# bobochow/adapt-image-models

Measured on AMD Instinct MI355X. Metric: clips/sec (8-frame 224^2 ViT-B/16 AIM fwd+bwd), higher is better.
Workload: dtype bf16; 1 GPU; BASELINE configs[1]: ViT-B/16 + AIM adapters, 8 frames 224^2, 64 clips/GPU, K400-shaped synthetic clips (400 random labels), fwd+bwd+AdamW; global_batch=64, frames=8, parallelism=dp1

## Files before the change

adapt-image-models_amd/backbone.py:

```python
import logging
import os
from collections import OrderedDict
from typing import Dict, List, Optional

import torch
from torch import nn

from . import ops
from .registry import BACKBONES

BF16, F32 = torch.bfloat16, torch.float32
_LOG = logging.getLogger("aim_amd")


def get_root_logger():
    return _LOG


class Adapter(nn.Module):

    def __init__(self, D_features: int, mlp_ratio: float = 0.25, skip_connect: bool = True):
        super().__init__()
        self.skip_connect = skip_connect
        hidden = int(D_features * mlp_ratio)
# ... 494 lines not shown
        ctx = dict(top=True, mean1c=mean1.view(BT, N)[:, 0].contiguous(), rstd1c=rstd1.view(BT, N)[:, 0].contiguous())
    elif save:
        ctx = {}
    if save:
        ctx.update(x=x, mean1=mean1, rstd1=rstd1, qkv=qkv, probs=probs, ta=ta, t_pre=t_pre, t_h=t_h, lam=lam,
                   oml=oml, ao=ao, lse=lse, sin=sin, s_pre=s_pre, s_h=s_h, x1=x1, mean2=mean2, rstd2=rstd2, xn=xn,
                   hcat_pre=hcat_pre, a_s=a_s, dms1=dms1, dms2=dms2)
    return x2, ctx


def _mlp_adapter_forward(x1, fz: _Frozen, dms2, N, save: bool, small_tile: bool = False):
    dev = x1.device
    M, D = x1.shape
    r, H4 = fz.r, 4 * D
    xn = _empty((M, D), BF16, dev)
    mean2, rstd2 = _empty((M,), F32, dev), _empty((M,), F32, dev)
    ops.layernorm_fwd(x1, fz.g2, fz.b2, M, D, D, y_bf16=xn, mean=mean2, rstd=rstd2)
    frag = _AUX_FRAG and M >= 1024 and not small_tile
    if frag:
        hcat_pre = ops.frag_buffer(M, H4 + r, dev) if save else None
    else:
        hcat_pre = _empty((M, H4 + r), BF16, dev) if (save or M < 1024 or small_tile) else None
    hcat = _empty((M, H4 + r), BF16, dev)
    ops.gemm(xn, fz.Wcat1, ops.EPI_ACT, hcat, bias=fz.bcat1, out2=hcat_pre, act=ops.ACT_QGELU, n_split=H4,
             act2=ops.ACT_GELU, at=dms2, ntok=N, aux_grad=_AUX_GRAD, aux_frag=frag and hcat_pre is not None,
             small_tile=small_tile)
    x2 = _empty((M, D), F32, dev)
    ops.gemm(hcat, fz.Wcat2, ops.EPI_F32, x2, bias=fz.bpr, resid=x1, vec=fz.b2row, ldv=0, bt=dms2, ntok=N, small_tile=small_tile)
    a_s = hcat[:, H4:] if save else None
    return x2, xn, mean2, rstd2, hcat_pre, a_s


def _mlp_adapter_backward(dyb, x_in, mean2, rstd2, xn, hcat_pre, a_s, dms2, fz: _Frozen, gm, N, fsum=None,
                          small_tile: bool = False):
    dev = dyb.device
    M, D = dyb.shape
    r, H4 = fz.r, 4 * D
    big_later: list = []
    if _DETACH_BIG:
        big_later.append(lambda: ops.wgrad(dyb, a_s, gm["D_fc2.weight"], gm["D_fc2.bias"], at=dms2, ntok=N))
    else:
        ops.wgrad(dyb, a_s, gm["D_fc2.weight"], gm["D_fc2.bias"], at=dms2, ntok=N)
    dcat = _empty((M, H4 + r), BF16, dev)
    ops.gemm(dyb, fz.WcatT2, ops.EPI_DACT, dcat, aux=hcat_pre, act=ops.ACT_QGELU, n_split=H4, act2=ops.ACT_GELU,
             at=dms2, ntok=N, aux_grad=_AUX_GRAD, aux_frag=_AUX_FRAG and dyb.shape[0] >= 1024 and not small_tile,
             reserve_cus=_DP_RESERVE, small_tile=small_tile)
    if _DETACH_BIG:
        big_later.append(lambda: ops.wgrad(dcat[:, H4:], xn, gm["D_fc1.weight"], gm["D_fc1.bias"]))
    else:
        ops.wgrad(dcat[:, H4:], xn, gm["D_fc1.weight"], gm["D_fc1.bias"])
    dxn = _empty((M, D), BF16, dev)
    ops.gemm(dcat, fz.WcatT1, ops.EPI_BF16, dxn, reserve_cus=_DP_RESERVE, small_tile=small_tile)
    dxb = _empty((M, D), BF16, dev)
    if fsum is not None:
        ops.layernorm_bwd_fsum(dxn, x_in, fz.g2, mean2, rstd2, dyb, dxb, fsum[0], fsum[1], M // N, N, D)
    else:
        ops.layernorm_bwd(dxn, x_in, fz.g2, mean2, rstd2, M, D, lddy=D, ldx=D, lddx=D, dres=dyb, dx_bf16=dxb)
    return dxb, big_later


def _adapter_bwd_small(dout_bf, ad: _AdapterW, a_in, pre, h, grads, rows, r, D, ar: _Arena, need_dx_bf16: bool, later: list):
    later.append(lambda: ops.wgrad(dout_bf, h, grads["D_fc2.weight"], grads["D_fc2.bias"]))
    dpre = ar.take((rows, r), BF16)
    ops.gemm(dout_bf, ad.W2T, ops.EPI_DACT, dpre, aux=pre, act=ops.ACT_GELU, aux_grad=_AUX_GRAD)
    later.append(lambda: ops.wgrad(dpre, a_in, grads["D_fc1.weight"], grads["D_fc1.bias"]))
    din = ar.take((rows, D), BF16 if need_dx_bf16 else F32)
    ops.gemm(dpre, ad.W1T, ops.EPI_BF16 if need_dx_bf16 else ops.EPI_F32, din)
    return din


def _block_backward(dyb, c, fz: _Frozen, adp: Dict[str, _AdapterW], grads, B, T, N, H, keep: Optional[list] = None):
    dev = dyb.device
    D = dyb.shape[1]
    BT = B * T
    M = BT * N
    r, H4 = fz.r, 4 * D
    top = bool(c.get("top"))
    fsum_in_ln = _FSUM_IN_LN and not top
    fpart = _empty((BT, ops.LN_FSUM_GROUPS, D), F32, dev) if fsum_in_ln else None
    if top:
        dx1b, big_later = _mlp_adapter_backward(dyb, c["x1"], c["mean2"], c["rstd2"], c["xn"], c["hcat_pre"], c["a_s"],
                                                c["dms2"][:1], fz, grads["MLP_Adapter"], 1, small_tile=True)
    else:
        dx1b, big_later = _mlp_adapter_backward(dyb, c["x1"], c["mean2"], c["rstd2"], c["xn"], c["hcat_pre"], c["a_s"], c["dms2"],
                                                fz, grads["MLP_Adapter"], N, fsum=(c["dms1"], fpart) if fsum_in_ln else None)
    later: list = big_later
    ar = _Arena(dev, 48 * BT * D + (1 << 16))
    with _Fork(dev, "bwd") as fork:
        dsv = ar.take((BT, D), F32)
        if fsum_in_ln:
            ops.frame_sum(fpart, None, dsv, BT, ops.LN_FSUM_GROUPS, D)
        elif top:
            ops.frame_sum(dx1b, c["dms1"][:1], dsv, BT, 1, D)
        else:
            ops.frame_sum(dx1b, c["dms1"], dsv, BT, N, D)
        dsv_b = ar.take((BT, D), BF16)
        ops.cast_bf16(dsv, dsv_b)
        dsin = _adapter_bwd_small(dsv_b, adp["S_Adapter"], c["sin"], c["s_pre"], c["s_h"], grads["S_Adapter"], BT, r,
                                  D, ar, need_dx_bf16=False, later=later)
        dcrs = ar.take((BT, D), BF16)
        ops.scale_rows(dsin, c["lam"], y=dcrs)
        dvx = ar.take((BT, D), BF16)
        ops.gemm(dcrs, fz.WoT, ops.EPI_BF16, dvx)
        dxt = ar.take((BT, D), BF16)
        ops.gemm(dvx, fz.WqkvT[:, 2 * D:], ops.EPI_BF16, dxt)
        dta = _adapter_bwd_small(dxt, adp["T_Adapter"], c["ta"], c["t_pre"], c["t_h"], grads["T_Adapter"], BT, r, D,
                                 ar, need_dx_bf16=True, later=later)
        dot = ar.take((BT, D), BF16)
        ops.gemm(dta, fz.WoT, ops.EPI_BF16, dot)
        if _LATE_JOIN:
            dqkv_cls = ar.take((BT, 3 * D), BF16)
            ops.cls_attn_bwd(c["qkv"], c["probs"], dot, dqkv_cls, B, T, N, H, compact=True)
            dxl_cls = ar.take((BT, D), F32)
            ops.gemm(dqkv_cls, fz.WqkvT, ops.EPI_F32, dxl_cls)
    if keep is None:
        keep = []
        fork.run_detached(later, keep)
        _Fork.join_detached(dev)
    else:
        fork.run_detached(later, keep)
    dqkv = _empty((M, 3 * D), BF16, dev)
    if top:
        dao = _empty((BT, D), BF16, dev)
        ops.gemm(dx1b, fz.WoT, ops.EPI_BF16, dao, af=c["oml"], ntok=1, small_tile=True)
        ops.attn_bwd_cls(c["qkv"], c["ao"], dao, c["lse"], dqkv, BT, N, H)
    else:
        dao = _empty((M, D), BF16, dev)
        ops.gemm(dx1b, fz.WoT, ops.EPI_BF16, dao, af=c["oml"], ntok=N, reserve_cus=_DP_RESERVE)
        delta = _empty((BT, H, N), F32, dev)
        ops.attn_bwd(c["qkv"], c["ao"], dao, c["lse"], delta, dqkv, BT, N, H)
    del dao
    if not _LATE_JOIN:
        fork.join()
        ops.cls_attn_bwd(c["qkv"], c["probs"], dot, dqkv, B, T, N, H)
    dxl = _empty((M, D), BF16, dev)
    ops.gemm(dqkv, fz.WqkvT, ops.EPI_BF16, dxl, reserve_cus=_DP_RESERVE)
    del dqkv
    if _LATE_JOIN:
        fork.join()
        ops.add_rows(dxl, N * D, dxl_cls)
    dxb = _empty((M, D), BF16, dev)
    if top:
        ops.layernorm_bwd(dxl, c["x"], fz.g1, c["mean1"], c["rstd1"], M, D, lddy=D, ldx=D, lddx=D, dx_bf16=dxb)
        ops.layernorm_bwd(dxl, c["x"], fz.g1, c["mean1c"], c["rstd1c"], BT, D, lddy=N * D, ldx=N * D, lddx=N * D, dres=dx1b,
                          lddres=D, dx_bf16=dxb)
    else:
        ops.layernorm_bwd(dxl, c["x"], fz.g1, c["mean1"], c["rstd1"], M, D, lddy=D, ldx=D, lddx=D, dres=dx1b, dx_bf16=dxb)
# ... 397 lines not shown
```

adapt-image-models_amd/csrc/wgrad.hip:

```cpp
#include "aim_common.h"
#include <stdlib.h>
#include "aim_kernels_internal.h"

namespace {

constexpr int MSTEP = 32;
constexpr int NST = 4;
constexpr int IMG = MSTEP * 128;
constexpr int OPER_BYTES = 4 * IMG;
constexpr int STAGE_BYTES = 2 * OPER_BYTES;
constexpr int TILE = 256;

__global__ __launch_bounds__(512) void wgrad_kernel(const bf16_t* __restrict__ G, int ldg, const bf16_t* __restrict__ A,
                                                    int lda, float* __restrict__ dW, int lddw, float* __restrict__ partial,
                                                    int M, int Nw, int Kw, int chunk, float* __restrict__ db,
                                                    float* __restrict__ bias_partial, const float* __restrict__ at, int ntok) {
    extern __shared__ __attribute__((aligned(16))) char smem_raw[];
    AIM_LDS char* smem = (AIM_LDS char*)smem_raw;
    AIM_LDS float* sAt = (AIM_LDS float*)(smem + NST * STAGE_BYTES);
    const int tiles_k = (Kw + TILE - 1) / TILE;
    const int tiles = ((Nw + TILE - 1) / TILE) * tiles_k;
    const int cidx = blockIdx.x / tiles, tix = blockIdx.x - cidx * tiles;
    const int tn = tix / tiles_k, tk = tix - tn * tiles_k;
    const int n0 = tn * TILE, k0 = tk * TILE;
    const int mbeg = cidx * chunk;
    const int mend = min(M, mbeg + chunk);
    if (mbeg >= mend) return;

    const int tid = threadIdx.x, lane = tid & 63;
    const int wave = __builtin_amdgcn_readfirstlane(tid >> 6);
    const int wn = wave >> 2, wk = wave & 3;
    const int frow = lane & 15, fq = lane >> 4;

    const bf16_t* Gb = G + (long long)mbeg * ldg + n0;
    const bf16_t* Ab = A + (long long)mbeg * lda + k0;
    const int rows = mend - mbeg;
    aim_rsrc_words rG = make_rsrc_words(Gb, ((long long)(rows - 1) * ldg + min(TILE, Nw - n0)) * 2);
    aim_rsrc_words rA = make_rsrc_words(Ab, ((long long)(rows - 1) * lda + min(TILE, Kw - k0)) * 2);

    const int srow = lane >> 3, schunk = (lane & 7) ^ srow;
    unsigned vg0[2], va0[2];
    AIM_LDS char* pdst[2];
#pragma unroll
    for (int j = 0; j < 2; ++j) {
        const int piece = wave * 2 + j;
        const int img = piece >> 2, rg = piece & 3;
        const int r = rg * 8 + srow;
        const int col = img * 64 + schunk * 8;
        vg0[j] = n0 + col < Nw ? (unsigned)((r * ldg + col) * 2) : AIM_OOB;
        va0[j] = k0 + col < Kw ? (unsigned)((r * lda + col) * 2) : AIM_OOB;
        pdst[j] = smem + img * IMG + rg * 1024;
    }
    const unsigned gstep = (unsigned)(MSTEP * ldg * 2), astep = (unsigned)(MSTEP * lda * 2);
    auto stage = [&](int buf, int ms) {
#pragma unroll
        for (int j = 0; j < 2; ++j) {
            stage_piece_asm(rG, pdst[j] + buf * STAGE_BYTES, vg0[j] + (unsigned)ms * gstep);
            stage_piece_asm(rA, pdst[j] + buf * STAGE_BYTES + OPER_BYTES, va0[j] + (unsigned)ms * astep);
        }
// ... 106 lines not shown
            f32x4 v[8];
#pragma unroll
            for (int j = 0; j < 8; ++j) v[j] = *(const f32x4*)(partial + (long long)(c + j) * total + idx);
#pragma unroll
            for (int j = 0; j < 8; ++j) acc += v[j];
        }
        for (; c < nchunks; ++c) acc += *(const f32x4*)(partial + (long long)c * total + idx);
        const int n = (int)(idx / Kw), k = (int)(idx - (long long)n * Kw);
        f32x4* o = (f32x4*)(dW + (long long)n * lddw + k);
        *o = *o + acc;
    }
    if (bias_partial) {
        const int n = blockIdx.x * 4 + (threadIdx.x >> 6), lane = threadIdx.x & 63;
        if (n < Nw) {
            float a = 0.f;
            for (int c = lane; c < nchunks; c += 64) a += bias_partial[(long long)c * Nw + n];
            a = wave_sum(a);
            if (lane == 0) db[n] += a;
        }
    }
}

__global__ __launch_bounds__(256) void wgrad_finish1_kernel(const float* __restrict__ partial, float* __restrict__ dW,
                                                            int lddw, int nchunks, int Nw, int Kw) {
    const long long idx = (long long)blockIdx.x * 256 + threadIdx.x;
    const long long total = (long long)Nw * Kw;
    if (idx >= total) return;
    float acc = 0.f;
    for (int c = 0; c < nchunks; ++c) acc += partial[(long long)c * total + idx];
    const int n = (int)(idx / Kw), k = (int)(idx - (long long)n * Kw);
    dW[(long long)n * lddw + k] += acc;
}

}

static int wgrad_chunks(int M, int tiles, int* chunk_out) {
    static const int target = [] { const char* e = getenv("AIM_WGRAD_WGS"); const int v = e ? atoi(e) : 256; return v > 0 ? v : 256; }();
    int nchunks = (target + tiles - 1) / tiles;
    const int maxchunks = (M + MSTEP - 1) / MSTEP;
    if (nchunks > maxchunks) nchunks = maxchunks;
    int chunk = (M + nchunks - 1) / nchunks;
    chunk = ((chunk + MSTEP - 1) / MSTEP) * MSTEP;
    if (chunk_out) *chunk_out = chunk;
    return (M + chunk - 1) / chunk;
}

extern "C" int64_t aim_wgrad_workspace_bytes(int M, int Nw, int Kw) {
    const int tiles = ((Nw + TILE - 1) / TILE) * ((Kw + TILE - 1) / TILE);
    const int nchunks = wgrad_chunks(M, tiles, nullptr);
    return nchunks > 1 ? (int64_t)nchunks * Nw * (Kw + 1) * 4 : 0;
}

extern "C" int aim_wgrad_bias_bf16(const aim_bf16* G, int ldg, const aim_bf16* A, int lda, float* dW, int lddw, float* db,
                                   const float* at, int ntok, int M, int Nw, int Kw, float* workspace, int64_t workspace_bytes,
                                   void* stream) {
    AIM_CHECK_ARG(M > 0 && Nw > 0 && Kw > 0 && (Nw % 8) == 0 && (Kw % 8) == 0, "wgrad: Nw/Kw must be positive multiples of 8 (Nw=%d Kw=%d)", Nw, Kw);
    AIM_CHECK_ARG((ldg % 8) == 0 && (lda % 8) == 0 && (lddw % 4) == 0, "wgrad: ldg/lda must be multiples of 8, lddw of 4");
    AIM_CHECK_ARG(G && A && dW, "wgrad: null pointer");
    AIM_CHECK_ARG(!at || (db && ntok > 0 && ntok <= 4096), "wgrad: row factors need db and 0 < ntok <= 4096");
    const int tiles = ((Nw + TILE - 1) / TILE) * ((Kw + TILE - 1) / TILE);
    int chunk = 0;
    const int nchunks = wgrad_chunks(M, tiles, &chunk);
    const int lds_bytes = NST * STAGE_BYTES + (at ? ((ntok * 4 + 15) & ~15) : 0);
    static bool attr_set = false;
    if (!attr_set) {
        (void)hipFuncSetAttribute((const void*)wgrad_kernel, hipFuncAttributeMaxDynamicSharedMemorySize, 160 * 1024);
        attr_set = true;
    }
    AIM_CHECK_ARG((long long)chunk * (ldg > lda ? ldg : lda) * 2 < 0x7fffffffLL, "wgrad: chunk too large");
    float* slab = (workspace && nchunks > 1 && workspace_bytes >= (int64_t)nchunks * Nw * (Kw + 1) * 4) ? workspace : nullptr;
    static const bool fuse_bias = [] { const char* e = getenv("AIM_WGRAD_FUSE_BIAS"); return !e || atoi(e) != 0; }();
    static const bool finish_v = [] { const char* e = getenv("AIM_WGRAD_FINISH_V"); return !e || atoi(e) != 0; }();
    float* bias_slab = (slab && db && fuse_bias) ? slab + (long long)nchunks * Nw * Kw : nullptr;
    if (db && nchunks > 1 && !bias_slab) {
        const int rc = aim_colsum_bf16(G, ldg, nullptr, at, ntok, db, M, Nw, nullptr, 0, stream);
        if (rc) return rc;
        db = nullptr;
    }
    hipLaunchKernelGGL(wgrad_kernel, dim3(tiles * nchunks), dim3(512), lds_bytes, (hipStream_t)stream,
                       (const bf16_t*)G, ldg, (const bf16_t*)A, lda, dW, lddw, slab, M, Nw, Kw, chunk, db, bias_slab, at, ntok);
    AIM_CHECK_LAUNCH("aim_wgrad_bf16");
    if (slab) {
        const long long total = (long long)Nw * Kw;
        unsigned fgrid = (unsigned)((total / 4 + 255) / 256);
        if (bias_slab && (unsigned)((Nw + 3) / 4) > fgrid) fgrid = (unsigned)((Nw + 3) / 4);
        if (finish_v || bias_slab)
            hipLaunchKernelGGL(wgrad_finish_kernel, dim3(fgrid), dim3(256), 0, (hipStream_t)stream,
                               slab, dW, lddw, nchunks, Nw, Kw, bias_slab, db);
        else
            hipLaunchKernelGGL(wgrad_finish1_kernel, dim3((unsigned)((total + 255) / 256)), dim3(256), 0, (hipStream_t)stream,
                               slab, dW, lddw, nchunks, Nw, Kw);
        AIM_CHECK_LAUNCH("aim_wgrad_bf16(finish)");
    }
    return 0;
}

extern "C" int aim_wgrad_bf16(const aim_bf16* G, int ldg, const aim_bf16* A, int lda, float* dW, int lddw, float* db,
                              int M, int Nw, int Kw, float* workspace, int64_t workspace_bytes, void* stream) {
    return aim_wgrad_bias_bf16(G, ldg, A, lda, dW, lddw, db, nullptr, 0, M, Nw, Kw, workspace, workspace_bytes, stream);
}
```

adapt-image-models_amd/lib.py:

```python
import ctypes
import os
from ctypes import POINTER, Structure, c_char_p, c_float, c_int, c_int32, c_int64, c_void_p

_HERE = os.path.dirname(os.path.abspath(__file__))
_LIB = None


class LibraryNotBuilt(RuntimeError):
    pass


def library_path() -> str:
    return os.environ.get("AIM_HIP_LIB") or os.path.join(_HERE, "libaim_hip.so")


class GemmArgs(Structure):
    _fields_ = [
        ("A", c_void_p), ("W", c_void_p), ("lda", c_int32), ("ldw", c_int32),
        ("strideA", c_int64), ("strideW", c_int64),
        ("M", c_int32), ("N", c_int32), ("K", c_int32),
        ("bias", c_void_p), ("resid", c_void_p), ("ldr", c_int32),
        ("af", c_void_p), ("at", c_void_p), ("vec", c_void_p), ("bt", c_void_p),
        ("ldv", c_int32), ("ntok", c_int32),
        ("aux", c_void_p), ("ldaux", c_int32),
        ("out", c_void_p), ("ldo", c_int32), ("out2", c_void_p), ("ldo2", c_int32),
        ("scale", c_float), ("act", c_int32), ("rs_bias_only", c_int32), ("n_split", c_int32), ("act2", c_int32),
        ("xrow", c_void_p), ("ldx", c_int32),
        ("reserve_cus", c_int32), ("probe", c_void_p), ("probe_cap", c_int32),
        ("wscale", c_void_p), ("aux_grad", c_int32), ("aux_frag", c_int32), ("row0", c_int32),
        ("small_tile", c_int32),
    ]


P = c_void_p
I = c_int
L = c_int64
F = c_float

SIGNATURES = {
    "aim_version": [],
    "aim_last_error": [],
    "aim_gemm_bf16": [POINTER(GemmArgs), I, I, P],
    "aim_gemm_fp8": [POINTER(GemmArgs), I, P],
    "aim_gemm_expsum_tiles": [I, I],
    "aim_wgrad_bf16": [P, I, P, I, P, I, P, I, I, I, P, L, P],
    "aim_wgrad_workspace_bytes": [I, I, I],
    "aim_wgrad_bias_bf16": [P, I, P, I, P, I, P, P, I, I, I, I, P, L, P],
    "aim_layernorm_fwd": [P, L, P, P, P, P, L, P, P, I, I, F, P],
    "aim_layernorm_fwd_fp8": [P, L, P, P, P, L, I, I, F, P],
    "aim_layernorm_fwd_x16": [P, L, P, P, P, P, P, L, I, I, F, P],
    "aim_layernorm_bwd": [P, I, L, P, L, P, P, P, P, I, L, P, P, L, P, P, I, I, P],
    "aim_layernorm_bwd_fsum": [P, L, P, L, P, P, P, P, P, L, P, P, I, I, I, I, P],
    "aim_attn_fwd": [P, P, P, I, I, I, P],
    "aim_attn_fwd_fp8": [P, P, P, I, I, I, P],
    "aim_attn_bwd": [P, P, P, P, P, P, I, I, I, P],
    "aim_attn_fwd_cls": [P, P, P, I, I, I, P],
    "aim_attn_bwd_cls": [P, P, P, P, P, I, I, I, P],
    "aim_cls_attn_fwd": [P, P, P, I, I, I, I, P],
    "aim_cls_attn_bwd": [P, P, P, P, I, I, I, I, I, P],
    "aim_tattn_fwd": [P, P, P, I, I, I, I, P],
    "aim_tattn_bwd": [P, P, P, P, I, I, I, I, P],
    "aim_add_bf16": [P, L, P, L, P, L, I, I, P],
    "aim_acc_bf16": [P, P, L, I, I, P],
    "aim_lambda_partials": [P, P, P, I, P],
    "aim_qk_cross": [P, P, I, P, I, I, I, F, P],
    "aim_lambda": [P, P, I, P, P, I, P, P, I, I, I, F, P],
    "aim_qk_border": [P, P, I, P, P, I, I, I, I, I, F, P],
    "aim_patchify": [P, I, P, P, P, I, I, I, I, I, I, P],
    "aim_patchify_blend": [P, I, P, P, P, I, I, I, I, I, I, P, I, F, F, I, I, I, I, P],
    "aim_embed_ln": [P, P, P, P, P, P, P, P, P, I, I, I, I, F, P],
    "aim_embed_bwd": [P, I, P, P, P, P, P, P, P, P, I, I, I, I, P, L, P],
    "aim_embed_bwd_workspace_bytes": [I, I, I, I],
    "aim_frame_sum": [P, I, P, P, I, I, I, P],
    "aim_colsum_bf16": [P, I, P, P, I, P, I, I, P, L, P],
    "aim_cast_bf16": [P, P, I, I, I, I, P],
    "aim_scale_rows": [P, P, P, P, I, I, P],
    "aim_add_rows_bf16": [P, L, P, I, I, P],
    "aim_adamw_flat": [P, P, P, P, L, F, F, F, F, F, I, F, P],
    "aim_head_fwd": [P, P, P, P, P, P, I, I, I, I, P],
    "aim_head_bwd": [P, P, P, P, P, P, P, I, I, I, I, P],
    "aim_ce_topk": [P, P, P, P, P, I, I, I, P],
    "aim_ce_soft": [P, P, P, P, P, P, I, I, P],
    "aim_cast_multi": [P, I, P],
    "aim_gemm_f32": [POINTER(GemmArgs), I, I, P],
    "aim_attn_fwd_f32": [P, P, I, I, I, P],
    "aim_cls_attn_fwd_f32": [P, L, P, I, I, I, P],
    "aim_lambda_f32": [P, I, P, P, I, P, P, I, I, I, F, P],
    "aim_patchify_f32": [P, I, P, P, P, I, I, I, I, I, I, P],
    "aim_patchify_blend_f32": [P, I, P, P, P, I, I, I, I, I, I, P, I, F, F, I, I, I, I, P],
    "aim_embed_ln_f32": [P, P, P, P, P, P, P, P, P, P, I, I, I, I, F, P],
    "aim_attn_bwd_f32_workspace_bytes": [I, I, I],
    "aim_attn_bwd_f32": [P, P, P, I, I, I, P, L, P],
    "aim_cls_attn_bwd_f32": [P, L, P, P, I, I, I, P],
    "aim_tattn_fwd_f32": [P, P, I, I, I, I, P],
    "aim_tattn_bwd_f32": [P, P, P, I, I, I, I, P],
    "aim_wgrad_f32_workspace_bytes": [I, I, I],
    "aim_wgrad_f32": [P, I, P, I, P, I, I, I, P, P, I, P, L, P],
    "aim_embed_nopre_fwd": [P, P, P, P, P, I, I, I, I, P],
    "aim_embed_nopre_bwd_workspace_bytes": [I, I, I, I],
    "aim_embed_nopre_bwd": [P, I, P, P, P, P, P, I, I, I, I, P, L, P],
    "aim_layernorm_gb_bwd_workspace_bytes": [I, I],
    "aim_layernorm_gb_bwd": [P, I, L, P, L, P, P, P, P, I, I, P, L, P],
}

ABI_VERSION = 9


def load_library():
    global _LIB
    if _LIB is not None:
        return _LIB
    path = library_path()
    if not os.path.exists(path):
        raise LibraryNotBuilt(
            f"{path} not found: build it with `python -c 'import __graft_entry__ as g; g.build()'` "
            f"(or `make -C adapt-image-models_amd/csrc`). There is no CPU fallback.")
    lib = ctypes.CDLL(path)
    for name, argtypes in SIGNATURES.items():
        fn = getattr(lib, name)
        fn.argtypes = argtypes
        fn.restype = c_char_p if name == "aim_last_error" else (c_int64 if name.endswith("_bytes") else c_int)
    if lib.aim_version() != ABI_VERSION:
        raise LibraryNotBuilt(f"{path}: ABI version {lib.aim_version()} != {ABI_VERSION}; rebuild")
    _LIB = lib
    return lib


def check(rc: int, what: str = ""):
    if rc != 0:
        msg = load_library().aim_last_error()
        raise RuntimeError(f"libaim_hip {what} failed (rc={rc}): {msg.decode() if msg else '?'}")
```

adapt-image-models_amd/ops.py:

```python
from ctypes import byref
from typing import Optional

import torch

from .lib import GemmArgs, check, load_library

EPI_BF16, EPI_ACT, EPI_DACT, EPI_F32, EPI_EXPSUM, EPI_ACT8, EPI_RES16 = 0, 1, 2, 3, 4, 5, 6
FP8 = torch.float8_e4m3fn
ACT_QGELU, ACT_GELU = 0, 1

BF16 = torch.bfloat16
F32 = torch.float32


_RAW_STREAM = getattr(torch._C, "_cuda_getCurrentRawStream", None)
_RAW_DEVICE = getattr(torch._C, "_cuda_getDevice", None)


def _stream() -> int:
    if _RAW_STREAM is not None:
        return _RAW_STREAM(_RAW_DEVICE())
    return torch.cuda.current_stream().cuda_stream


class KernelTimer:

    def __init__(self, min_flops: float = 1e10):
        self.min_flops = min_flops
        self.enabled = False
        self.records = []

    def start(self):
        self.records, self.enabled = [], True

    def stop(self):
        self.enabled = False

    def summary(self):
# ... 152 lines not shown
    check(load_library().aim_layernorm_fwd_fp8(x.data_ptr(), ldx, gamma.data_ptr(), beta.data_ptr(), y8.data_ptr(),
                                               D if ldy is None else ldy, rows, D, eps, _stream()), "aim_layernorm_fwd_fp8")


def layernorm_fwd_x16(x, gamma, beta, rows, D, ldx, *, y_bf16=None, y_f32=None, y8=None, ldy=None, eps: float = 1e-5):
    _chk(x, BF16, "x"); _chk(gamma, F32, "gamma"); _chk(beta, F32, "beta"); _chk(y_bf16, BF16, "y_bf16"); _chk(y_f32, F32, "y_f32")
    if y8 is not None and (y8.element_size() != 1 or not y8.is_cuda):
        raise TypeError("y8: expected a GPU fp8 (1-byte) tensor")
    check(load_library().aim_layernorm_fwd_x16(x.data_ptr(), ldx, gamma.data_ptr(), beta.data_ptr(), _p(y_bf16), _p(y_f32), _p(y8),
                                               D if ldy is None else ldy, rows, D, eps, _stream()), "aim_layernorm_fwd_x16")


def attn_fwd_fp8(qkv, out8, BT, N, H, lse=None):
    _chk(qkv, BF16, "qkv"); _chk(lse, F32, "lse")
    if out8.element_size() != 1 or not out8.is_cuda:
        raise TypeError("out8: expected a GPU fp8 (1-byte) tensor")
    check(load_library().aim_attn_fwd_fp8(qkv.data_ptr(), out8.data_ptr(), _p(lse), BT, N, H, _stream()), "aim_attn_fwd_fp8")


def expsum_tiles(M: int, N: int) -> int:
    return load_library().aim_gemm_expsum_tiles(M, N)


def wgrad(g: torch.Tensor, a: torch.Tensor, dw: torch.Tensor, db: Optional[torch.Tensor] = None, at=None, ntok: int = 0):
    _chk(g, BF16, "g"); _chk(a, BF16, "a"); _chk(dw, F32, "dw"); _chk(db, F32, "db"); _chk(at, F32, "at")
    assert g.shape[0] == a.shape[0] and dw.shape == (g.shape[1], a.shape[1])
    lib = load_library()
    nbytes = lib.aim_wgrad_workspace_bytes(g.shape[0], g.shape[1], a.shape[1])
    ws = torch.empty(nbytes // 4, dtype=F32, device=g.device) if nbytes else None
    check(lib.aim_wgrad_bias_bf16(g.data_ptr(), g.stride(0), a.data_ptr(), a.stride(0), dw.data_ptr(), dw.stride(0), _p(db),
                                  _p(at), ntok, g.shape[0], g.shape[1], a.shape[1], _p(ws), nbytes, _stream()), "aim_wgrad_bias_bf16")


def layernorm_fwd(x, gamma, beta, rows, D, ldx, *, y_bf16=None, y_f32=None, ldy=None, mean=None, rstd=None,
                  eps: float = 1e-5):
    _chk(x, F32, "x"); _chk(gamma, F32, "gamma"); _chk(beta, F32, "beta")
    _chk(y_bf16, BF16, "y_bf16"); _chk(y_f32, F32, "y_f32"); _chk(mean, F32, "mean"); _chk(rstd, F32, "rstd")
    check(load_library().aim_layernorm_fwd(x.data_ptr(), ldx, gamma.data_ptr(), beta.data_ptr(), _p(y_bf16),
                                           _p(y_f32), D if ldy is None else ldy, _p(mean), _p(rstd), rows, D,
                                           eps, _stream()), "aim_layernorm_fwd")


def layernorm_bwd(dy, x, gamma, mean, rstd, rows, D, *, lddy, ldx, lddx, dres=None, dx=None, dx_bf16=None,
                  dgamma=None, dbeta=None, lddres=None):
    for n_, t_ in (("x", x), ("gamma", gamma), ("mean", mean), ("rstd", rstd),
                   ("dx", dx), ("dgamma", dgamma), ("dbeta", dbeta)):
        _chk(t_, F32, n_)
    _chk(dx_bf16, BF16, "dx_bf16")
    _chk(dy, dy.dtype if dy.dtype in (F32, BF16) else F32, "dy")
    if dres is not None:
        _chk(dres, dres.dtype if dres.dtype in (F32, BF16) else F32, "dres")
    check(load_library().aim_layernorm_bwd(dy.data_ptr(), int(dy.dtype == BF16), lddy, x.data_ptr(), ldx, gamma.data_ptr(),
                                           mean.data_ptr(), rstd.data_ptr(), _p(dres),
                                           int(dres is not None and dres.dtype == BF16),
                                           lddx if lddres is None else lddres, _p(dx), _p(dx_bf16), lddx,
                                           _p(dgamma), _p(dbeta), rows, D, _stream()), "aim_layernorm_bwd")


LN_FSUM_GROUPS = 13


def layernorm_bwd_fsum(dy, x, gamma, mean, rstd, dres, dx_bf16, w, partial, frames, ntok, D):
    _chk(dy, BF16, "dy"); _chk(dres, BF16, "dres"); _chk(dx_bf16, BF16, "dx_bf16")
    for n_, t_ in (("x", x), ("gamma", gamma), ("mean", mean), ("rstd", rstd), ("w", w), ("partial", partial)):
        _chk(t_, F32, n_)
    assert partial.numel() >= frames * LN_FSUM_GROUPS * D
# ... 417 lines not shown
```

include/aim_kernels.h:

```cpp
#ifndef AIM_KERNELS_H
#define AIM_KERNELS_H

#include <stdint.h>

#ifdef __cplusplus
extern "C" {
#endif

typedef uint16_t aim_bf16;

#define AIM_ABI_VERSION 9

int aim_version(void);
const char* aim_last_error(void);

enum {
    AIM_EPI_BF16 = 0,
    AIM_EPI_ACT = 1,
    AIM_EPI_DACT = 2,
    AIM_EPI_F32 = 3,
    AIM_EPI_EXPSUM = 4,
    AIM_EPI_ACT8 = 5,
    AIM_EPI_RES16 = 6
};
enum { AIM_ACT_QGELU = 0, AIM_ACT_GELU = 1 };

typedef struct aim_gemm_args {
    const aim_bf16* A;
    const aim_bf16* W;
    int32_t lda, ldw;
    int64_t strideA, strideW;
    int32_t M, N, K;
    const float* bias;
    const float* resid;
    int32_t ldr;
    const float* af;
    const float* at;
    const float* vec;
    const float* bt;
    int32_t ldv, ntok;
    const aim_bf16* aux;
    int32_t ldaux;
    void* out;  int32_t ldo;
    void* out2; int32_t ldo2;
    float scale;
    int32_t act;
    int32_t rs_bias_only;
    int32_t n_split, act2;
    const aim_bf16* xrow;
    int32_t ldx;
    int32_t reserve_cus;
    void* probe;
    int32_t probe_cap;
    const float* wscale;
    int32_t aux_grad;
    int32_t aux_frag;
    int32_t row0;
    int32_t small_tile;
} aim_gemm_args;

int aim_gemm_bf16(const aim_gemm_args* args, int epilogue, int batch, void* stream);

int aim_gemm_fp8(const aim_gemm_args* args, int epilogue, void* stream);
int aim_gemm_expsum_tiles(int M, int N);

int aim_wgrad_bf16(const aim_bf16* G, int ldg, const aim_bf16* A, int lda, float* dW, int lddw,
                   float* db, int M, int Nw, int Kw,
                   float* workspace ,
                   int64_t workspace_bytes, void* stream);
int64_t aim_wgrad_workspace_bytes(int M, int Nw, int Kw);
int aim_wgrad_bias_bf16(const aim_bf16* G, int ldg, const aim_bf16* A, int lda, float* dW, int lddw, float* db,
                        const float* at, int ntok, int M, int Nw, int Kw, float* workspace, int64_t workspace_bytes, void* stream);

int aim_layernorm_fwd(const float* x, int64_t ldx, const float* gamma, const float* beta,
                      aim_bf16* y_bf16, float* y_f32, int64_t ldy, float* mean, float* rstd,
                      int rows, int D, float eps, void* stream);
int aim_layernorm_fwd_fp8(const float* x, int64_t ldx, const float* gamma, const float* beta, uint8_t* y_fp8,
                          int64_t ldy, int rows, int D, float eps, void* stream);
int aim_layernorm_fwd_x16(const aim_bf16* x, int64_t ldx, const float* gamma, const float* beta, aim_bf16* y_bf16,
                          float* y_f32, uint8_t* y_fp8, int64_t ldy, int rows, int D, float eps, void* stream);
int aim_layernorm_bwd(const void* dy, int dy_is_bf16 , int64_t lddy,
                      const float* x, int64_t ldx, const float* gamma,
                      const float* mean, const float* rstd, const void* dres, int dres_is_bf16,
                      int64_t lddres , float* dx,
                      aim_bf16* dx_bf16, int64_t lddx, float* dgamma, float* dbeta,
                      int rows, int D, void* stream);
int aim_layernorm_bwd_fsum(const aim_bf16* dy, int64_t lddy, const float* x, int64_t ldx, const float* gamma,
                           const float* mean, const float* rstd, const aim_bf16* dres, aim_bf16* dx_bf16, int64_t lddx,
                           const float* w, float* fsum_partial, int groups, int frames, int ntok, int D, void* stream);

int aim_attn_fwd(const aim_bf16* qkv, aim_bf16* out, float* lse, int BT, int N, int H, void* stream);
int aim_attn_fwd_fp8(const aim_bf16* qkv, uint8_t* out_fp8, float* lse, int BT, int N, int H, void* stream);
int aim_attn_bwd(const aim_bf16* qkv, const aim_bf16* out, const aim_bf16* dout, const float* lse,
                 float* delta , aim_bf16* dqkv, int BT, int N, int H,
                 void* stream);
int aim_attn_fwd_cls(const aim_bf16* qkv, aim_bf16* out_cls, float* lse_cls, int BT, int N, int H, void* stream);
int aim_attn_bwd_cls(const aim_bf16* qkv, const aim_bf16* out_cls, const aim_bf16* dout_cls, const float* lse_cls,
                     aim_bf16* dqkv, int BT, int N, int H, void* stream);

int aim_cls_attn_fwd(const aim_bf16* qkv, aim_bf16* out_cls, float* probs, int B, int T, int N, int H,
                     void* stream);
int aim_cls_attn_bwd(const aim_bf16* qkv, const float* probs, const aim_bf16* dout_cls, aim_bf16* dqkv, int compact,
                     int B, int T, int N, int H, void* stream);

int aim_tattn_fwd(const aim_bf16* qkv, aim_bf16* out, float* probs, int B, int T, int N, int H, void* stream);
// ... 95 lines not shown
```

Baseline: 1365 clips/s.

## Group small adapter weight-gradient GEMMs into one launch and rebalance wgrad chunking

Adds a grouped small-M wgrad kernel (64x64 tiles, up to 8 problems per launch, fused bias reduction). The adapter weight gradients in each block backward (S/T adapters, and the MLP adapter in the top block) are queued and issued as grouped launches instead of one launch per GEMM. The large wgrad path now sizes its M-chunk count from the device CU count and spreads remainder steps evenly, replacing the fixed 256-workgroup target. The aim is to cut launch overhead and poor occupancy on tiny GEMMs. The trade-off is a more complex dispatch path and different split-K partitioning for the large wgrads.

```diff
diff --git a/adapt-image-models_amd/backbone.py b/adapt-image-models_amd/backbone.py
--- a/adapt-image-models_amd/backbone.py
+++ b/adapt-image-models_amd/backbone.py
@@ -550,12 +550,15 @@
 
 
 def _mlp_adapter_backward(dyb, x_in, mean2, rstd2, xn, hcat_pre, a_s, dms2, fz: _Frozen, gm, N, fsum=None,
-                          small_tile: bool = False):
+                          small_tile: bool = False, small: Optional[list] = None):
     dev = dyb.device
     M, D = dyb.shape
     r, H4 = fz.r, 4 * D
     big_later: list = []
-    if _DETACH_BIG:
+    grouped = small is not None and _DETACH_BIG and M <= ops.WGRAD_SMALL_M
+    if grouped:
+        small.append((dyb, a_s, gm["D_fc2.weight"], gm["D_fc2.bias"], dms2, N))
+    elif _DETACH_BIG:
         big_later.append(lambda: ops.wgrad(dyb, a_s, gm["D_fc2.weight"], gm["D_fc2.bias"], at=dms2, ntok=N))
     else:
         ops.wgrad(dyb, a_s, gm["D_fc2.weight"], gm["D_fc2.bias"], at=dms2, ntok=N)
@@ -563,7 +566,9 @@
     ops.gemm(dyb, fz.WcatT2, ops.EPI_DACT, dcat, aux=hcat_pre, act=ops.ACT_QGELU, n_split=H4, act2=ops.ACT_GELU,
              at=dms2, ntok=N, aux_grad=_AUX_GRAD, aux_frag=_AUX_FRAG and dyb.shape[0] >= 1024 and not small_tile,
              reserve_cus=_DP_RESERVE, small_tile=small_tile)
-    if _DETACH_BIG:
+    if grouped:
+        small.append((dcat[:, H4:], xn, gm["D_fc1.weight"], gm["D_fc1.bias"], None, 0))
+    elif _DETACH_BIG:
         big_later.append(lambda: ops.wgrad(dcat[:, H4:], xn, gm["D_fc1.weight"], gm["D_fc1.bias"]))
     else:
         ops.wgrad(dcat[:, H4:], xn, gm["D_fc1.weight"], gm["D_fc1.bias"])
@@ -577,14 +582,23 @@
     return dxb, big_later
 
 
-def _adapter_bwd_small(dout_bf, ad: _AdapterW, a_in, pre, h, grads, rows, r, D, ar: _Arena, need_dx_bf16: bool, later: list):
-    later.append(lambda: ops.wgrad(dout_bf, h, grads["D_fc2.weight"], grads["D_fc2.bias"]))
+def _adapter_bwd_small(dout_bf, ad: _AdapterW, a_in, pre, h, grads, rows, r, D, ar: _Arena, need_dx_bf16: bool, small: list):
+    small.append((dout_bf, h, grads["D_fc2.weight"], grads["D_fc2.bias"], None, 0))
     dpre = ar.take((rows, r), BF16)
     ops.gemm(dout_bf, ad.W2T, ops.EPI_DACT, dpre, aux=pre, act=ops.ACT_GELU, aux_grad=_AUX_GRAD)
-    later.append(lambda: ops.wgrad(dpre, a_in, grads["D_fc1.weight"], grads["D_fc1.bias"]))
+    small.append((dpre, a_in, grads["D_fc1.weight"], grads["D_fc1.bias"], None, 0))
     din = ar.take((rows, D), BF16 if need_dx_bf16 else F32)
     ops.gemm(dpre, ad.W1T, ops.EPI_BF16 if need_dx_bf16 else ops.EPI_F32, din)
     return din
+
+
+def _queue_small_wgrads(small: list, later: list):
+    few = [q for q in small if q[0].shape[0] <= ops.WGRAD_SMALL_M]
+    for q in small:
+        if q[0].shape[0] > ops.WGRAD_SMALL_M:
+            later.append(lambda q=q: ops.wgrad(q[0], q[1], q[2], q[3], at=q[4], ntok=q[5]))
+    for i in range(0, len(few), ops.WGRAD_GROUP_MAX):
+        later.append(lambda g=few[i:i + ops.WGRAD_GROUP_MAX]: ops.wgrad_group(g))
 
 
 def _block_backward(dyb, c, fz: _Frozen, adp: Dict[str, _AdapterW], grads, B, T, N, H, keep: Optional[list] = None):
@@ -596,9 +610,10 @@
     top = bool(c.get("top"))
     fsum_in_ln = _FSUM_IN_LN and not top
     fpart = _empty((BT, ops.LN_FSUM_GROUPS, D), F32, dev) if fsum_in_ln else None
+    small: list = []
     if top:
         dx1b, big_later = _mlp_adapter_backward(dyb, c["x1"], c["mean2"], c["rstd2"], c["xn"], c["hcat_pre"], c["a_s"],
-                                                c["dms2"][:1], fz, grads["MLP_Adapter"], 1, small_tile=True)
+                                                c["dms2"][:1], fz, grads["MLP_Adapter"], 1, small_tile=True, small=small)
     else:
         dx1b, big_later = _mlp_adapter_backward(dyb, c["x1"], c["mean2"], c["rstd2"], c["xn"], c["hcat_pre"], c["a_s"], c["dms2"],
                                                 fz, grads["MLP_Adapter"], N, fsum=(c["dms1"], fpart) if fsum_in_ln else None)
@@ -615,7 +630,7 @@
         dsv_b = ar.take((BT, D), BF16)
         ops.cast_bf16(dsv, dsv_b)
         dsin = _adapter_bwd_small(dsv_b, adp["S_Adapter"], c["sin"], c["s_pre"], c["s_h"], grads["S_Adapter"], BT, r,
-                                  D, ar, need_dx_bf16=False, later=later)
+                                  D, ar, need_dx_bf16=False, small=small)
         dcrs = ar.take((BT, D), BF16)
         ops.scale_rows(dsin, c["lam"], y=dcrs)
         dvx = ar.take((BT, D), BF16)
@@ -623,7 +638,7 @@
         dxt = ar.take((BT, D), BF16)
         ops.gemm(dvx, fz.WqkvT[:, 2 * D:], ops.EPI_BF16, dxt)
         dta = _adapter_bwd_small(dxt, adp["T_Adapter"], c["ta"], c["t_pre"], c["t_h"], grads["T_Adapter"], BT, r, D,
-                                 ar, need_dx_bf16=True, later=later)
+                                 ar, need_dx_bf16=True, small=small)
         dot = ar.take((BT, D), BF16)
         ops.gemm(dta, fz.WoT, ops.EPI_BF16, dot)
         if _LATE_JOIN:
@@ -631,6 +646,7 @@
             ops.cls_attn_bwd(c["qkv"], c["probs"], dot, dqkv_cls, B, T, N, H, compact=True)
             dxl_cls = ar.take((BT, D), F32)
             ops.gemm(dqkv_cls, fz.WqkvT, ops.EPI_F32, dxl_cls)
+    _queue_small_wgrads(small, later)
     if keep is None:
         keep = []
         fork.run_detached(later, keep)
diff --git a/adapt-image-models_amd/csrc/wgrad.hip b/adapt-image-models_amd/csrc/wgrad.hip
--- a/adapt-image-models_amd/csrc/wgrad.hip
+++ b/adapt-image-models_amd/csrc/wgrad.hip
@@ -11,9 +11,11 @@
 constexpr int STAGE_BYTES = 2 * OPER_BYTES;
 constexpr int TILE = 256;
 
+__host__ __device__ inline int wgrad_chunk_begin(int c, int base, int rem) { return MSTEP * (c * base + (c < rem ? c : rem)); }
+
 __global__ __launch_bounds__(512) void wgrad_kernel(const bf16_t* __restrict__ G, int ldg, const bf16_t* __restrict__ A,
                                                     int lda, float* __restrict__ dW, int lddw, float* __restrict__ partial,
-                                                    int M, int Nw, int Kw, int chunk, float* __restrict__ db,
+                                                    int M, int Nw, int Kw, int base, int rem, float* __restrict__ db,
                                                     float* __restrict__ bias_partial, const float* __restrict__ at, int ntok) {
     extern __shared__ __attribute__((aligned(16))) char smem_raw[];
     AIM_LDS char* smem = (AIM_LDS char*)smem_raw;
@@ -23,8 +25,8 @@
     const int cidx = blockIdx.x / tiles, tix = blockIdx.x - cidx * tiles;
     const int tn = tix / tiles_k, tk = tix - tn * tiles_k;
     const int n0 = tn * TILE, k0 = tk * TILE;
-    const int mbeg = cidx * chunk;
-    const int mend = min(M, mbeg + chunk);
+    const int mbeg = wgrad_chunk_begin(cidx, base, rem);
+    const int mend = min(M, wgrad_chunk_begin(cidx + 1, base, rem));
     if (mbeg >= mend) return;
 
     const int tid = threadIdx.x, lane = tid & 63;
@@ -197,43 +199,264 @@
     dW[(long long)n * lddw + k] += acc;
 }
 
-}
-
-static int wgrad_chunks(int M, int tiles, int* chunk_out) {
-    static const int target = [] { const char* e = getenv("AIM_WGRAD_WGS"); const int v = e ? atoi(e) : 256; return v > 0 ? v : 256; }();
-    int nchunks = (target + tiles - 1) / tiles;
-    const int maxchunks = (M + MSTEP - 1) / MSTEP;
-    if (nchunks > maxchunks) nchunks = maxchunks;
-    int chunk = (M + nchunks - 1) / nchunks;
-    chunk = ((chunk + MSTEP - 1) / MSTEP) * MSTEP;
-    if (chunk_out) *chunk_out = chunk;
-    return (M + chunk - 1) / chunk;
+constexpr int SMALL_MAX = 8;
+constexpr int SMALL_M = 1024;
+constexpr int STILE = 64;
+constexpr int SNST = 6;
+constexpr int SSTAGE = 2 * IMG;
+
+struct WgradGroup {
+    aim_wgrad_problem p[SMALL_MAX];
+    int tile0[SMALL_MAX + 1];
+    int count;
+};
+
+__global__ __launch_bounds__(256) void wgrad_small_kernel(const WgradGroup grp) {
+    __shared__ __attribute__((aligned(16))) char smem_raw[SNST * SSTAGE + SMALL_M * 4];
+    AIM_LDS char* smem = (AIM_LDS char*)smem_raw;
+    AIM_LDS float* sF = (AIM_LDS float*)(smem + SNST * SSTAGE);
+    int pi = 0;
+#pragma unroll
+    for (int i = 1; i < SMALL_MAX; ++i)
+        if (i < grp.count && (int)blockIdx.x >= grp.tile0[i]) pi = i;
+    const aim_wgrad_problem& P = grp.p[pi];
+    const bf16_t* G = (const bf16_t*)P.G;
+    const bf16_t* A = (const bf16_t*)P.A;
+    const int ldg = P.ldg, lda = P.lda, M = P.M, Nw = P.Nw, Kw = P.Kw;
+    const int tix = (int)blockIdx.x - grp.tile0[pi];
+    const int tiles_k = (Kw + STILE - 1) / STILE;
+    const int tn = tix / tiles_k, tk = tix - tn * tiles_k;
+    const int n0 = tn * STILE, k0 = tk * STILE;
+
+    const int tid = threadIdx.x, lane = tid & 63;
+    const int wave = __builtin_amdgcn_readfirstlane(tid >> 6);
+    const int wn = wave >> 1, wk = wave & 1;
+    const int frow = lane & 15, fq = lane >> 4;
+
+    const bool do_bias = P.db != nullptr && tk == 0;
+    if (do_bias) {
+        const float* at = P.at;
+        const int ntok = P.ntok;
+        for (int m = tid; m < SMALL_M; m += 256) sF[m] = m < M ? (at ? at[m % ntok] : 1.0f) : 0.f;
+        asm volatile("s_waitcnt vmcnt(0) lgkmcnt(0)" ::: "memory");
+    }
+
+    aim_rsrc_words rG = make_rsrc_words(G + n0, ((long long)(M - 1) * ldg + min(STILE, Nw - n0)) * 2);
+    aim_rsrc_words rA = make_rsrc_words(A + k0, ((long long)(M - 1) * lda + min(STILE, Kw - k0)) * 2);
+    const int srow = lane >> 3, schunk = (lane & 7) ^ srow;
+    const int r = wave * 8 + srow, col = schunk * 8;
+    const unsigned vg0 = n0 + col < Nw ? (unsigned)((r * ldg + col) * 2) : AIM_OOB;
+    const unsigned va0 = k0 + col < Kw ? (unsigned)((r * lda + col) * 2) : AIM_OOB;
+    AIM_LDS char* pdst = smem + wave * 1024;
+    const unsigned gstep = (unsigned)(MSTEP * ldg * 2), astep = (unsigned)(MSTEP * lda * 2);
+    const int nsteps = (M + MSTEP - 1) / MSTEP;
+    auto stage = [&](int buf, int ms) {
+        const bool live = ms < nsteps;
+        stage_piece_asm(rG, pdst + buf * SSTAGE, live ? vg0 + (unsigned)ms * gstep : AIM_OOB);
+        stage_piece_asm(rA, pdst + buf * SSTAGE + IMG, live ? va0 + (unsigned)ms * astep : AIM_OOB);
+    };
+
+    f32x4 acc[2][2];
+#pragma unroll
+    for (int i = 0; i < 2; ++i)
+#pragma unroll
+        for (int j = 0; j < 2; ++j) acc[i][j] = f32x4{0.f, 0.f, 0.f, 0.f};
+
+    auto frag = [&](const AIM_LDS char* img, int c0) -> bf16x8 {
+        const int ch = (c0 >> 3) + ((frow & 3) >> 1), half8 = (frow & 1) * 8;
+        const int r0 = fq * 4 + (frow >> 2);
+        const bf16x4 a = lds_read_tr4(img + swz_off(r0, ch) + half8);
+        const bf16x4 b = lds_read_tr4(img + swz_off(r0 + 16, ch) + half8);
+        bf16x8 f;
+#pragma unroll
+        for (int e = 0; e < 4; ++e) {
+            f[e] = a[e];
+            f[4 + e] = b[e];
+        }
+        return f;
+    };
+
+    float bs[8] = {0.f, 0.f, 0.f, 0.f, 0.f, 0.f, 0.f, 0.f};
+    const int bcg = tid & 7, brow = tid >> 3;
+#pragma unroll
+    for (int st = 0; st < SNST - 1; ++st) stage(st, st);
+    for (int ms = 0; ms < nsteps; ++ms) {
+        asm volatile("s_waitcnt vmcnt(8)" ::: "memory");
+        static_assert(2 * (SNST - 2) == 8, "vmcnt literal above");
+        __builtin_amdgcn_s_barrier();
+        stage((ms + SNST - 1) % SNST, ms + SNST - 1);
+        const AIM_LDS char* sG = smem + (ms % SNST) * SSTAGE;
+        const AIM_LDS char* sA = sG + IMG;
+        if (do_bias) {
+            const bf16x8 v = lds_read8(sG + swz_off(brow, bcg));
+            const float f = sF[ms * MSTEP + brow];
+#pragma unroll
+            for (int e = 0; e < 8; ++e) bs[e] += f * (float)v[e];
+        }
+        bf16x8 gf[2], af[2];
+#pragma unroll
+        for (int j = 0; j < 2; ++j) af[j] = frag(sA, wk * 32 + j * 16);
+#pragma unroll
+        for (int i = 0; i < 2; ++i) gf[i] = frag(sG, wn * 32 + i * 16);
+#pragma unroll
+        for (int i = 0; i < 2; ++i)
+#pragma unroll
+            for (int j = 0; j < 2; ++j)
+                acc[i][j] = __builtin_amdgcn_mfma_f32_16x16x32_bf16(af[j], gf[i], acc[i][j], 0, 0, 0);
+    }
+    asm volatile("s_waitcnt vmcnt(0)" ::: "memory");
+    if (do_bias) {
+        __syncthreads();
+        AIM_LDS float* red = (AIM_LDS float*)smem;
+#pragma unroll
+        for (int e = 0; e < 8; ++e) red[brow * STILE + bcg * 8 + e] = bs[e];
+        __syncthreads();
+        if (tid < STILE && n0 + tid < Nw) {
+            float v = 0.f;
+#pragma unroll
+            for (int rr = 0; rr < MSTEP; ++rr) v += red[rr * STILE + tid];
+            P.db[n0 + tid] += v;
+        }
+    }
+    float* dW = P.dW;
+    const int lddw = P.lddw;
+#pragma unroll
+    for (int i = 0; i < 2; ++i)
+#pragma unroll
+        for (int j = 0; j < 2; ++j) {
+            const int n = n0 + wn * 32 + i * 16 + frow;
+            const int k = k0 + wk * 32 + j * 16 + fq * 4;
+            if (n >= Nw || k >= Kw) continue;
+            f32x4* o = (f32x4*)(dW + (long long)n * lddw + k);
+            *o = *o + acc[i][j];
+        }
+}
+
+}
+
+static bool wgrad_route_on() {
+    static const bool on = [] { const char* e = getenv("AIM_WGRAD_ROUTE"); return !e || atoi(e) != 0; }();
+    return on;
+}
+
+struct WgradPlan {
+    bool small;
+    int tiles, nchunks;
+    int base, rem;
+    int chunk;
+};
+
+static WgradPlan wgrad_plan(int M, int Nw, int Kw, int cus) {
+    WgradPlan p;
+    const int steps = (M + MSTEP - 1) / MSTEP;
+    if (wgrad_route_on() && M <= SMALL_M) {
+        p.small = true;
+        p.tiles = ((Nw + STILE - 1) / STILE) * ((Kw + STILE - 1) / STILE);
+        p.nchunks = 1;
+        p.base = steps;
+        p.rem = 0;
+        p.chunk = steps * MSTEP;
+        return p;
+    }
+    p.small = false;
+    p.tiles = ((Nw + TILE - 1) / TILE) * ((Kw + TILE - 1) / TILE);
+    static const int env_target = [] { const char* e = getenv("AIM_WGRAD_WGS"); const int v = e ? atoi(e) : 0; return v > 0 ? v : 0; }();
+    if (!wgrad_route_on()) {
+        const int target = env_target ? env_target : 256;
+        int nchunks = (target + p.tiles - 1) / p.tiles;
+        if (nchunks > steps) nchunks = steps;
+        int chunk = (M + nchunks - 1) / nchunks;
+        chunk = ((chunk + MSTEP - 1) / MSTEP) * MSTEP;
+        p.chunk = chunk;
+        p.base = chunk / MSTEP;
+        p.rem = 0;
+        p.nchunks = (M + chunk - 1) / chunk;
+        return p;
+    }
+    const int target = env_target && env_target < cus ? env_target : cus;
+    int nchunks = target / p.tiles;
+    if (nchunks < 1) nchunks = 1;
+    if (nchunks > steps) nchunks = steps;
+    p.nchunks = nchunks;
+    p.base = steps / nchunks;
+    p.rem = steps % nchunks;
+    p.chunk = (p.base + (p.rem ? 1 : 0)) * MSTEP;
+    return p;
+}
+
+static int64_t wgrad_plan_bytes(const WgradPlan& p, int Nw, int Kw) {
+    return p.nchunks > 1 ? (int64_t)p.nchunks * Nw * (Kw + 1) * 4 : 0;
+}
+
+extern "C" int aim_wgrad_plan(int M, int Nw, int Kw, int cus, int* chunk, int* nchunks, int* tiles, int64_t* workspace_bytes) {
+    AIM_CHECK_ARG(M > 0 && Nw > 0 && Kw > 0, "wgrad_plan: M, Nw, Kw must be positive");
+    const WgradPlan p = wgrad_plan(M, Nw, Kw, cus > 0 ? cus : aim_device_cus());
+    if (chunk) *chunk = p.chunk;
+    if (nchunks) *nchunks = p.nchunks;
+    if (tiles) *tiles = p.tiles;
+    if (workspace_bytes) *workspace_bytes = wgrad_plan_bytes(p, Nw, Kw);
+    return 0;
+}
+
+extern "C" int aim_wgrad_plan_rows(int M, int Nw, int Kw, int cus, int c, int* mbeg, int* mend) {
+    AIM_CHECK_ARG(M > 0 && Nw > 0 && Kw > 0 && mbeg && mend, "wgrad_plan_rows: bad arguments");
+    const WgradPlan p = wgrad_plan(M, Nw, Kw, cus > 0 ? cus : aim_device_cus());
+    AIM_CHECK_ARG(c >= 0 && c < p.nchunks, "wgrad_plan_rows: chunk %d of %d", c, p.nchunks);
+    const int b = wgrad_chunk_begin(c, p.base, p.rem), e = wgrad_chunk_begin(c + 1, p.base, p.rem);
+    *mbeg = b < M ? b : M;
+    *mend = e < M ? e : M;
+    return 0;
 }
 
 extern "C" int64_t aim_wgrad_workspace_bytes(int M, int Nw, int Kw) {
-    const int tiles = ((Nw + TILE - 1) / TILE) * ((Kw + TILE - 1) / TILE);
-    const int nchunks = wgrad_chunks(M, tiles, nullptr);
-    return nchunks > 1 ? (int64_t)nchunks * Nw * (Kw + 1) * 4 : 0;
+    if (M <= 0 || Nw <= 0 || Kw <= 0) return 0;
+    return wgrad_plan_bytes(wgrad_plan(M, Nw, Kw, aim_device_cus()), Nw, Kw);
+}
+
+static int wgrad_check_problem(const aim_wgrad_problem& q) {
+    AIM_CHECK_ARG(q.M > 0 && q.Nw > 0 && q.Kw > 0 && (q.Nw % 8) == 0 && (q.Kw % 8) == 0, "wgrad: Nw/Kw must be positive multiples of 8 (Nw=%d Kw=%d)", q.Nw, q.Kw);
+    AIM_CHECK_ARG((q.ldg % 8) == 0 && (q.lda % 8) == 0 && (q.lddw % 4) == 0, "wgrad: ldg/lda must be multiples of 8, lddw of 4");
+    AIM_CHECK_ARG(q.G && q.A && q.dW, "wgrad: null pointer");
+    AIM_CHECK_ARG(!q.at || (q.db && q.ntok > 0 && q.ntok <= 4096), "wgrad: row factors need db and 0 < ntok <= 4096");
+    return 0;
+}
+
+extern "C" int aim_wgrad_group_bf16(const aim_wgrad_problem* problems, int count, void* stream) {
+    AIM_CHECK_ARG(problems && count >= 1 && count <= SMALL_MAX, "wgrad_group: 1..%d problems (count=%d)", SMALL_MAX, count);
+    WgradGroup grp = {};
+    grp.count = count;
+    int grid = 0;
+    for (int i = 0; i < count; ++i) {
+        const aim_wgrad_problem& q = problems[i];
+        if (wgrad_check_problem(q)) return 1;
+        AIM_CHECK_ARG(q.M <= SMALL_M, "wgrad_group: problem %d has M = %d > %d rows", i, q.M, SMALL_M);
+        AIM_CHECK_ARG(((long long)q.M * (q.ldg > q.lda ? q.ldg : q.lda) + 64) * 2 < 0x7fffffffLL, "wgrad_group: rows too long");
+        grp.p[i] = q;
+        grp.tile0[i] = grid;
+        grid += ((q.Nw + STILE - 1) / STILE) * ((q.Kw + STILE - 1) / STILE);
+    }
+    for (int i = count; i <= SMALL_MAX; ++i) grp.tile0[i] = grid;
+    hipLaunchKernelGGL(wgrad_small_kernel, dim3(grid), dim3(256), 0, (hipStream_t)stream, grp);
+    AIM_CHECK_LAUNCH("aim_wgrad_group_bf16");
+    return 0;
 }
 
 extern "C" int aim_wgrad_bias_bf16(const aim_bf16* G, int ldg, const aim_bf16* A, int lda, float* dW, int lddw, float* db,
                                    const float* at, int ntok, int M, int Nw, int Kw, float* workspace, int64_t workspace_bytes,
                                    void* stream) {
-    AIM_CHECK_ARG(M > 0 && Nw > 0 && Kw > 0 && (Nw % 8) == 0 && (Kw % 8) == 0, "wgrad: Nw/Kw must be positive multiples of 8 (Nw=%d Kw=%d)", Nw, Kw);
-    AIM_CHECK_ARG((ldg % 8) == 0 && (lda % 8) == 0 && (lddw % 4) == 0, "wgrad: ldg/lda must be multiples of 8, lddw of 4");
-    AIM_CHECK_ARG(G && A && dW, "wgrad: null pointer");
-    AIM_CHECK_ARG(!at || (db && ntok > 0 && ntok <= 4096), "wgrad: row factors need db and 0 < ntok <= 4096");
-    const int tiles = ((Nw + TILE - 1) / TILE) * ((Kw + TILE - 1) / TILE);
-    int chunk = 0;
-    const int nchunks = wgrad_chunks(M, tiles, &chunk);
+    aim_wgrad_problem q = {G, A, dW, db, at, ldg, lda, lddw, M, Nw, Kw, ntok, 0};
+    if (wgrad_check_problem(q)) return 1;
+    const WgradPlan plan = wgrad_plan(M, Nw, Kw, aim_device_cus());
+    if (plan.small) return aim_wgrad_group_bf16(&q, 1, stream);
+    const int tiles = plan.tiles, nchunks = plan.nchunks;
     const int lds_bytes = NST * STAGE_BYTES + (at ? ((ntok * 4 + 15) & ~15) : 0);
     static bool attr_set = false;
     if (!attr_set) {
         (void)hipFuncSetAttribute((const void*)wgrad_kernel, hipFuncAttributeMaxDynamicSharedMemorySize, 160 * 1024);
         attr_set = true;
     }
-    AIM_CHECK_ARG((long long)chunk * (ldg > lda ? ldg : lda) * 2 < 0x7fffffffLL, "wgrad: chunk too large");
-    float* slab = (workspace && nchunks > 1 && workspace_bytes >= (int64_t)nchunks * Nw * (Kw + 1) * 4) ? workspace : nullptr;
+    AIM_CHECK_ARG((long long)plan.chunk * (ldg > lda ? ldg : lda) * 2 < 0x7fffffffLL, "wgrad: chunk too large");
+    float* slab = (workspace && nchunks > 1 && workspace_bytes >= wgrad_plan_bytes(plan, Nw, Kw)) ? workspace : nullptr;
     static const bool fuse_bias = [] { const char* e = getenv("AIM_WGRAD_FUSE_BIAS"); return !e || atoi(e) != 0; }();
     static const bool finish_v = [] { const char* e = getenv("AIM_WGRAD_FINISH_V"); return !e || atoi(e) != 0; }();
     float* bias_slab = (slab && db && fuse_bias) ? slab + (long long)nchunks * Nw * Kw : nullptr;
@@ -243,7 +466,7 @@
         db = nullptr;
     }
     hipLaunchKernelGGL(wgrad_kernel, dim3(tiles * nchunks), dim3(512), lds_bytes, (hipStream_t)stream,
-                       (const bf16_t*)G, ldg, (const bf16_t*)A, lda, dW, lddw, slab, M, Nw, Kw, chunk, db, bias_slab, at, ntok);
+                       (const bf16_t*)G, ldg, (const bf16_t*)A, lda, dW, lddw, slab, M, Nw, Kw, plan.base, plan.rem, db, bias_slab, at, ntok);
     AIM_CHECK_LAUNCH("aim_wgrad_bf16");
     if (slab) {
         const long long total = (long long)Nw * Kw;
diff --git a/adapt-image-models_amd/lib.py b/adapt-image-models_amd/lib.py
--- a/adapt-image-models_amd/lib.py
+++ b/adapt-image-models_amd/lib.py
@@ -32,6 +32,14 @@
     ]
 
 
+class WgradProblem(Structure):
+    _fields_ = [
+        ("G", c_void_p), ("A", c_void_p), ("dW", c_void_p), ("db", c_void_p), ("at", c_void_p),
+        ("ldg", c_int32), ("lda", c_int32), ("lddw", c_int32), ("M", c_int32), ("Nw", c_int32), ("Kw", c_int32),
+        ("ntok", c_int32), ("reserved", c_int32),
+    ]
+
+
 P = c_void_p
 I = c_int
 L = c_int64
@@ -46,6 +54,9 @@
     "aim_wgrad_bf16": [P, I, P, I, P, I, P, I, I, I, P, L, P],
     "aim_wgrad_workspace_bytes": [I, I, I],
     "aim_wgrad_bias_bf16": [P, I, P, I, P, I, P, P, I, I, I, I, P, L, P],
+    "aim_wgrad_group_bf16": [P, I, P],
+    "aim_wgrad_plan": [I, I, I, I, P, P, P, P],
+    "aim_wgrad_plan_rows": [I, I, I, I, I, P, P],
     "aim_layernorm_fwd": [P, L, P, P, P, P, L, P, P, I, I, F, P],
     "aim_layernorm_fwd_fp8": [P, L, P, P, P, L, I, I, F, P],
     "aim_layernorm_fwd_x16": [P, L, P, P, P, P, P, L, I, I, F, P],
@@ -103,7 +114,7 @@
     "aim_layernorm_gb_bwd": [P, I, L, P, L, P, P, P, P, I, I, P, L, P],
 }
 
-ABI_VERSION = 9
+ABI_VERSION = 10
 
 
 def load_library():
diff --git a/adapt-image-models_amd/ops.py b/adapt-image-models_amd/ops.py
--- a/adapt-image-models_amd/ops.py
+++ b/adapt-image-models_amd/ops.py
@@ -1,9 +1,10 @@
+import os
 from ctypes import byref
 from typing import Optional
 
 import torch
 
-from .lib import GemmArgs, check, load_library
+from .lib import GemmArgs, WgradProblem, check, load_library
 
 EPI_BF16, EPI_ACT, EPI_DACT, EPI_F32, EPI_EXPSUM, EPI_ACT8, EPI_RES16 = 0, 1, 2, 3, 4, 5, 6
 FP8 = torch.float8_e4m3fn
@@ -222,6 +223,44 @@
                                   _p(at), ntok, g.shape[0], g.shape[1], a.shape[1], _p(ws), nbytes, _stream()), "aim_wgrad_bias_bf16")
 
 
+WGRAD_SMALL_M, WGRAD_GROUP_MAX = 1024, 8
+WGRAD_ROUTE = os.environ.get("AIM_WGRAD_ROUTE", "1") != "0"
+
+
+def wgrad_plan(M: int, Nw: int, Kw: int, cus: int = 0):
+    from ctypes import c_int, c_int64
+    lib = load_library()
+    chunk, nchunks, tiles, nbytes = c_int(), c_int(), c_int(), c_int64()
+    check(lib.aim_wgrad_plan(M, Nw, Kw, cus, byref(chunk), byref(nchunks), byref(tiles), byref(nbytes)), "aim_wgrad_plan")
+    rows = []
+    for c in range(nchunks.value):
+        b, e = c_int(), c_int()
+        check(lib.aim_wgrad_plan_rows(M, Nw, Kw, cus, c, byref(b), byref(e)), "aim_wgrad_plan_rows")
+        rows.append((b.value, e.value))
+    return dict(chunk=chunk.value, nchunks=nchunks.value, tiles=tiles.value, workspace_bytes=nbytes.value, rows=rows)
+
+
+def wgrad_group(problems):
+    if not problems:
+        return
+    if not WGRAD_ROUTE:
+        for g, a, dw, db, at, ntok in problems:
+            wgrad(g, a, dw, db, at=at, ntok=ntok)
+        return
+    if len(problems) > WGRAD_GROUP_MAX:
+        raise ValueError(f"wgrad_group: at most {WGRAD_GROUP_MAX} problems per launch")
+    arr = (WgradProblem * len(problems))()
+    for q, (g, a, dw, db, at, ntok) in zip(arr, problems):
+        _chk(g, BF16, "g"); _chk(a, BF16, "a"); _chk(dw, F32, "dw"); _chk(db, F32, "db"); _chk(at, F32, "at")
+        assert g.shape[0] == a.shape[0] and dw.shape == (g.shape[1], a.shape[1])
+        if g.shape[0] > WGRAD_SMALL_M:
+            raise ValueError(f"wgrad_group: {g.shape[0]} rows; a grouped problem has at most {WGRAD_SMALL_M}")
+        q.G, q.A, q.dW, q.db, q.at = g.data_ptr(), a.data_ptr(), dw.data_ptr(), _p(db), _p(at)
+        q.ldg, q.lda, q.lddw = g.stride(0), a.stride(0), dw.stride(0)
+        q.M, q.Nw, q.Kw, q.ntok = g.shape[0], g.shape[1], a.shape[1], ntok
+    check(load_library().aim_wgrad_group_bf16(arr, len(problems), _stream()), "aim_wgrad_group_bf16")
+
+
 def layernorm_fwd(x, gamma, beta, rows, D, ldx, *, y_bf16=None, y_f32=None, ldy=None, mean=None, rstd=None,
                   eps: float = 1e-5):
     _chk(x, F32, "x"); _chk(gamma, F32, "gamma"); _chk(beta, F32, "beta")
diff --git a/include/aim_kernels.h b/include/aim_kernels.h
--- a/include/aim_kernels.h
+++ b/include/aim_kernels.h
@@ -9,7 +9,7 @@
 
 typedef uint16_t aim_bf16;
 
-#define AIM_ABI_VERSION 9
+#define AIM_ABI_VERSION 10
 
 int aim_version(void);
 const char* aim_last_error(void);
@@ -71,6 +71,17 @@
 int64_t aim_wgrad_workspace_bytes(int M, int Nw, int Kw);
 int aim_wgrad_bias_bf16(const aim_bf16* G, int ldg, const aim_bf16* A, int lda, float* dW, int lddw, float* db,
                         const float* at, int ntok, int M, int Nw, int Kw, float* workspace, int64_t workspace_bytes, void* stream);
+typedef struct aim_wgrad_problem {
+    const aim_bf16* G;
+    const aim_bf16* A;
+    float* dW;
+    float* db;
+    const float* at;
+    int32_t ldg, lda, lddw, M, Nw, Kw, ntok, reserved;
+} aim_wgrad_problem;
+int aim_wgrad_group_bf16(const aim_wgrad_problem* problems, int count, void* stream);
+int aim_wgrad_plan(int M, int Nw, int Kw, int cus, int* chunk, int* nchunks, int* tiles, int64_t* workspace_bytes);
+int aim_wgrad_plan_rows(int M, int Nw, int Kw, int cus, int c, int* mbeg, int* mend);
 
 int aim_layernorm_fwd(const float* x, int64_t ldx, const float* gamma, const float* beta,
                       aim_bf16* y_bf16, float* y_f32, int64_t ldy, float* mean, float* rstd,
```

Measured after the change: 1371 clips/s, median of 6. Within noise of the previous version (+0.4%).
